# xXCoffeeColaXc/WeatherConverter

Hardware: AMD Instinct MI355X
Metric: 256x256 images/sec (T=1000 DDPM sample) (higher is better)
Workload: dtype fp32-class (f16x3: 2-piece fp16 split MFMA, fp32 accumulate); 1 GPU; DDPM reverse sampling, UNet config.yaml @ 256px, 16 images/GPU, T=1000, 127 timed steps from t=999; global_batch=16, image_size=256, parallelism=single GPU, devices=1, hip_graph=True, stream_groups=2, x_finite=True

## Files before the change

### weatherconverter_amd/csrc/wc_wino.hip

```cpp
#include <stdlib.h>

#include "wc_x6.hpp"

#ifndef WC_ABL
#define WC_ABL 0
#endif
#ifndef WC_WINO_SCALAR
#define WC_WINO_SCALAR 0
#endif

namespace {

using namespace wcx6;

constexpr int NT = 256;

WC_DEVICE void wino_lds16(__amdgpu_buffer_rsrc_t srd, void* dst, unsigned voff, int soff) {
    __builtin_amdgcn_raw_ptr_buffer_load_lds(srd, (__attribute__((address_space(3))) void*)dst, 16, voff, soff, 0, 0);
}

struct WDev {
    const float* src0;
    int C0, ldc0;
    const float* scale;
    const float* shift;
    const float* src1;
    int C1, ldc1;
    int B, H, W, N;
    const void* w;
    const float* bias;
    const float* temb;
    int temb_ld;
    const float* res;
    int ldres;
    float* out;
    int ldo;
    int nck0, nck1;
    int a_exp;
    const float* abound;
    const float* wsinv;
    float* absmax;
    float* gn_part;
    int gn_ncb, gn_sw, gn_c0, gn_np64;
    int tiles_x, tiles_y, ntiles_n;
    const unsigned char* vpre;
    long vimg;
    const float* gb_x;
    int gb_ldx, gb_silu;
    const float* gb_sc0;
    const float* gb_sh0;
    const float* gb_gamma;
    const float* gb_beta;
    float* gb_part;
    float* gb_part3;
};

WC_DEVICE float wino_silu_grad(float y) {
    const float s = 1.0f / (1.0f + __expf(-y));
    return s * (1.0f + y * (1.0f - s));
}

constexpr int VPL = WC_SINGLE16 ? 8 : 16;

template <int TH, int BN, int MB = 2, int NW = 4, bool VP = false>
struct WTile {
    static constexpr int NT = 64 * NW;
    static constexpr int WAVES_N = BN / 32;
    static constexpr int WAVES_M = NW / WAVES_N;
    static_assert(WAVES_N * WAVES_M == NW && WAVES_M * 4 * MB == TH, "each wave owns 4 MB rows x 8 tiles x 32 channels");
    static constexpr int PBN = BN > 128 ? 128 : BN;
    static constexpr int HR = TH + 2;
    static constexpr int PSTR = HR * 128 + (VP ? 0 : 16);
    static constexpr int DPIECES = VPL * HR * 8 / 64;
    static_assert(!VP || VPL * HR * 8 == DPIECES * 64, "VP: the halo stage is a whole number of 1-KiB pieces");
    static constexpr int DPW = (DPIECES + NW - 1) / NW;
    static constexpr int HSTAGE = 16 * PSTR;
    static constexpr int CPSTR = TH * 128 + 16;
    static constexpr int CSTAGE = 8 * CPSTR;
    static constexpr int ITEMS = HR * 16;
    static constexpr int I_PER_T = (ITEMS + NT - 1) / NT;
    static constexpr int C_PER_T = TH * 16 * 4 / NT;
    static constexpr int BSTEP = PBN * 64;
    static constexpr int STEPS = 12;
};

WC_DEVICE int wg_grp(int r) { return ((r >= 4 && r < 12) || (r >= 16 && r < 20) || r >= 28) ? 1 : 0; }
WC_DEVICE int wg_idx(int r) { return r < 4 ? r : r < 12 ? r - 4 : r < 20 ? r - 8 : r < 28 ? r - 12 : r - 16; }
WC_DEVICE int wg_row(int r) { return 2 * wg_grp(r) + (wg_idx(r) >> 3); }
WC_DEVICE int wg_tile(int r) { return wg_idx(r) & 7; }

template <int TH, int BN, int PRO, bool RES, int MB = 2, int NW = 4>
__global__ __launch_bounds__(64 * NW) __attribute__((amdgpu_waves_per_eu(MB == 4 ? 1 : 2, MB == 4 ? 1 : 2)))
void conv3x3_wino_kernel(WDev p) {
    static_assert((PRO == 2 || PRO == 0 || PRO == 3) && !(PRO == 0 && RES),
                  "GN+SiLU (+ residual), pre-split GN+SiLU (+ residual) or one raw segment");
    constexpr bool VP = PRO == 3;
    using T = WTile<TH, BN, MB, NW, VP>;
    constexpr int NT = T::NT;
    extern __shared__ __attribute__((aligned(16))) unsigned char smem[];
    unsigned char* const cbase = smem + 2 * T::HSTAGE;

    const int tid = threadIdx.x;
    const int lane = tid & 63;
    const int wave = tid >> 6;
    const int wm = wave / T::WAVES_N;
    const int wn = wave % T::WAVES_N;

    const int nblk = gridDim.x;
    int bid = blockIdx.x;
    {
        int q = nblk / 8, r = nblk % 8, xcd = bid % 8;
        bid = (xcd < r ? xcd * (q + 1) : r * (q + 1) + (xcd - r) * q) + bid / 8;
    }
    const int tile_n = bid % p.ntiles_n;
    int tt = bid / p.ntiles_n;
    const int txi = tt % p.tiles_x;
    tt /= p.tiles_x;
    const int tyi = tt % p.tiles_y;
    const int b = tt / p.tiles_y;
    const int y0 = tyi * TH, x0 = txi * 16, n0 = tile_n * BN;

    int s_exp = p.a_exp;
    if ((RES || PRO == 0) && p.abound) {
        const float bnd = p.abound[b];
        const int e = (int)((__float_as_uint(bnd) >> 23) & 0xffu) - 127;
        if (bnd > 0.f) s_exp = min(s_exp, (PRO == 0 ? 12 : 13) - e);
        s_exp = max(s_exp, -100);
    }
    const float ascale = ldexpf(1.0f, s_exp), ainv = ldexpf(1.0f, -s_exp);
    const int S0 = T::STEPS * p.nck0;
    const int S = S0 + (RES ? p.nck1 : 0);
    constexpr bool RI = RES && (T::C_PER_T <= 2 || MB == 4);
    const int nri = RI ? min(p.nck0, p.nck1) : 0;
    const int ntail = RES ? p.nck1 - nri : 0;
    constexpr int WPT = T::PBN / 32;
    const unsigned wtile = (unsigned)(tile_n * (BN / T::PBN) + wn / WPT) * (unsigned)(S * T::BSTEP);

    const __amdgpu_buffer_rsrc_t srd0 = make_srd(p.src0);
    const __amdgpu_buffer_rsrc_t srd1 = make_srd(RES ? p.src1 : p.src0);
    const __amdgpu_buffer_rsrc_t srdw = make_srd(p.w);
    const __amdgpu_buffer_rsrc_t srdsc = make_srd(PRO == 2 ? p.scale : p.src0);
    const __amdgpu_buffer_rsrc_t srdsh = make_srd(PRO == 2 ? p.shift : p.src0);
    const __amdgpu_buffer_rsrc_t srdv = make_srd(VP ? (const void*)(p.vpre + (long)b * p.vimg) : (const void*)p.src0);
    unsigned voff[VP ? T::DPW : 1];
    if constexpr (VP) {
#pragma unroll
        for (int i = 0; i < T::DPW; ++i) {
            const int f = (wave + NW * i) * 64 + lane;
            const int P = f / (T::HR * 8), r = (f >> 3) % T::HR, tl = f & 7;
            const int y = y0 - 1 + r;
            voff[i] = (unsigned)y < (unsigned)p.H ? (unsigned)(((P * p.H + y) * (p.W / 2) + (x0 >> 1) + tl) * 16) : OOB;
        }
    }
    const int vchunk = VPL * p.H * (p.W / 2) * 16;
    auto dma_halo = [&](int c, int hs) {
        if constexpr (VP) {
            unsigned char* dst = smem + hs * T::HSTAGE + wave * 1024;
#pragma unroll
            for (int i = 0; i < T::DPW; ++i)
                if (T::DPIECES % NW == 0 || wave + NW * i < T::DPIECES)
                    wino_lds16(srdv, dst + i * NW * 1024, voff[i], c * vchunk);
        }
    };

    const int q = tid & 3;
    int hbase[T::I_PER_T];
    unsigned hin[T::I_PER_T];
    int hwr[T::I_PER_T];
    const int hpx = p.ldc0 * 4;
#pragma unroll
    for (int j = 0; j < T::I_PER_T; ++j) {
        const int i = tid + NT * j;
        const int hrow = i >> 4, tp = (i >> 2) & 3;
        const bool valid = i < T::ITEMS;
        const int iy = y0 - 1 + hrow;
        hin[j] = 0;
#pragma unroll
        for (int k = 0; k < 6; ++k) {
            const int ix = x0 - 1 + 4 * tp + k;
            const bool inb = valid && (unsigned)iy < (unsigned)p.H && (unsigned)ix < (unsigned)p.W;
            hin[j] |= (inb ? 1u : 0u) << k;
        }
        hbase[j] = (((b * p.H + iy) * p.W + x0 - 1 + 4 * tp) * p.ldc0 + 4 * q) * 4;
        hwr[j] = valid ? (q >> 1) * T::PSTR + (hrow * 8 + 2 * tp) * 16 + (q & 1) * 8 : -1;
    }
    f32x4 rh[T::I_PER_T][6];
    f32x4 rsc, rsh;
    auto load_ss = [&](int c) {
        if constexpr (PRO == 2) {
            const unsigned o = (unsigned)(b * p.C0 + c * 16 + 4 * q) * 4u;
            rsc = bload_f4(srdsc, o);
            rsh = bload_f4(srdsh, o);
        }
    };
    auto load_slot = [&](int j, int c) {
#pragma unroll
        for (int k = 0; k < 6; ++k)
            rh[j][k] = bload_f4s(srd0, ((hin[j] >> k) & 1u) ? (unsigned)(hbase[j] + k * hpx) : OOB, c * 64);
    };
    auto load_halo = [&](int c) {
        if constexpr (VP) return;
#pragma unroll
        for (int j = 0; j < T::I_PER_T; ++j) load_slot(j, c);
        load_ss(c);
    };
#if WC_WINO_SCALAR
    const float cu = -1.4426950408889634f * ainv;
    auto prologue = [&](int j, int k0, int k1) {
        if constexpr (PRO == 2) {
            if (j == 0 && k0 == 0) {
                rsc = rsc * ascale;
                rsh = rsh * ascale;
            }
        }
        auto act = [&](f32x4 a) {
#pragma unroll
            for (int e = 0; e < 4; ++e) {
                float v;
                if constexpr (PRO == 2) {
                    const float ap = __builtin_fmaf(a[e], rsc[e], rsh[e]);
                    const float r = __builtin_amdgcn_rcpf(1.0f + __builtin_amdgcn_exp2f(ap * cu));
                    v = ap * r;
                } else {
                    v = a[e] * ascale;
                }
                a[e] = v;
            }
            return a;
        };
#pragma unroll
        for (int k = k0; k < k1; ++k) {
            const f32x4 zero = {0.f, 0.f, 0.f, 0.f};
#if WC_WINO_SCALAR == 2
            rh[j][k] = ((hin[j] >> k) & 1u) ? act(rh[j][k]) : zero;
#else
            const f32x4 a = act(rh[j][k]);
            rh[j][k] = ((hin[j] >> k) & 1u) ? a : zero;
#endif
        }
    };
#else
    auto prologue = [&](int j, int k0, int k1) {
#pragma unroll
        for (int k = k0; k < k1; ++k) {
            f32x4 a = rh[j][k];
            if constexpr (PRO == 2 && !(WC_ABL & 2)) {
                a = a * rsc + rsh;
                if constexpr (!(WC_ABL & 1)) {
                    a.x = silu_fast(a.x); a.y = silu_fast(a.y);
                    a.z = silu_fast(a.z); a.w = silu_fast(a.w);
                }
            }
            rh[j][k] = ((hin[j] >> k) & 1u) ? a * ascale : f32x4{0.f, 0.f, 0.f, 0.f};
        }
    };
#endif
    auto transform = [&](int j, int t, int hs, int p0 = 0, int p1 = 4) {
        if (hwr[j] < 0) return;
        unsigned char* base = smem + hs * T::HSTAGE + hwr[j] + t * 16;
        const f32x4 d0 = rh[j][2 * t], d1 = rh[j][2 * t + 1], d2 = rh[j][2 * t + 2], d3 = rh[j][2 * t + 3];
#if WC_WINO_SCALAR
        f32x4 V[4];
#pragma unroll
        for (int e = 0; e < 4; ++e) {
            V[0][e] = d0[e] - d2[e];
            V[1][e] = d1[e] + d2[e];
            V[2][e] = d2[e] - d1[e];
            V[3][e] = d1[e] - d3[e];
        }
#else
        const f32x4 V[4] = {d0 - d2, d1 + d2, d2 - d1, d1 - d3};
#endif
#pragma unroll
        for (int pos = p0; pos < p1; ++pos) {
            u32x2 a0, a1;
            split2_f16(V[pos], a0, a1);
            unsigned char* d = base + pos * 2 * T::PSTR;
            *reinterpret_cast<u32x2*>(d) = a0;
            *reinterpret_cast<u32x2*>(d + 8 * T::PSTR) = a1;
        }
    };
    auto write_items = [&](int hs) {
        if constexpr (VP) return;
#pragma unroll
        for (int j = 0; j < T::I_PER_T; ++j) {
            prologue(j, 0, 6);
            transform(j, 0, hs);
            transform(j, 1, hs);
        }
    };

    f32x4 rc[2][RES ? T::C_PER_T : 1];
    const int cpx = (tid >> 2) & 15, crow0 = tid >> 6;
    const unsigned coff0 = (unsigned)(((b * p.H + y0 + crow0) * p.W + x0 + cpx) * p.ldc1 + 4 * q);
    const unsigned cstep = (unsigned)(NW * p.W * p.ldc1);
    const int cwr0 = (cpx & 1) * 2 * T::CPSTR + (q >> 1) * T::CPSTR + (crow0 * 8 + (cpx >> 1)) * 16 + (q & 1) * 8;
    auto load_centre = [&](auto P, int c, bool live = true) {
        constexpr int PV = decltype(P)::value;
        const unsigned v = live ? coff0 * 4u : OOB;
#pragma unroll
        for (int j = 0; j < T::C_PER_T; ++j)
            rc[PV][j] = bload_f4s(srd1, v, (int)(((unsigned)j * cstep + (unsigned)c * 16u) * 4u));
    };
    auto write_centre = [&](auto P, int cs) {
        constexpr int PV = decltype(P)::value;
        unsigned char* base = cbase + cs * T::CSTAGE + cwr0;
        const float sg = (cpx & 1) ? -ascale : ascale;
#pragma unroll
        for (int j = 0; j < T::C_PER_T; ++j) {
            u32x2 a0, a1;
            split2_f16(rc[PV][j] * sg, a0, a1);
            unsigned char* d = base + j * NW * 8 * 16;
            *reinterpret_cast<u32x2*>(d) = a0;
            *reinterpret_cast<u32x2*>(d + 4 * T::CPSTR) = a1;
        }
    };

    const int l32 = lane & 31;
    const int half = lane >> 5;
    int abase[MB];
#pragma unroll
    for (int mb = 0; mb < MB; ++mb) abase[mb] = ((4 * MB * wm + 4 * mb + wg_row(l32)) * 8 + wg_tile(l32)) * 16;
    const unsigned wlane = (unsigned)(half * T::PBN * 16 + ((wn % WPT) * 32 + l32) * 16);

    u32x4 wreg[3][2];
    auto load_w = [&](int set, int st) {
        int s = st < S0 ? st : S0 + nri + (st - S0);
        s = s < S ? s : S - 1;
        const int off = (int)(wtile + (unsigned)s * T::BSTEP);
#pragma unroll
        for (int pc = 0; pc < 2; ++pc) wreg[set][pc] = bload_u4s(srdw, wlane + (unsigned)(pc * 2 * T::PBN * 16), off);
    };
    u32x4 wres[2];
    auto load_wres = [&](int r) {
        const int s = S0 + r < S ? S0 + r : S - 1;
        const int off = (int)(wtile + (unsigned)s * T::BSTEP);
#pragma unroll
        for (int pc = 0; pc < 2; ++pc) wres[pc] = bload_u4s(srdw, wlane + (unsigned)(pc * 2 * T::PBN * 16), off);
    };

    f32x16 acc[4][MB];
#pragma unroll
    for (int i = 0; i < 4; ++i)
#pragma unroll
        for (int j = 0; j < MB; ++j)
#pragma unroll
            for (int r = 0; r < 16; ++r) acc[i][j][r] = 0.f;

    u32x4 fa[2][MB][2];
    auto read_a = [&](int fs, int hs, int dy, int pos) {
        const unsigned char* ha = smem + hs * T::HSTAGE + (pos * 2 + half) * T::PSTR + dy * 128;
#pragma unroll
        for (int mb = 0; mb < MB; ++mb)
#pragma unroll
            for (int pc = 0; pc < 2; ++pc)
                fa[fs][mb][pc] = *reinterpret_cast<const u32x4*>(ha + pc * 8 * T::PSTR + abase[mb]);
    };
    auto mfma_a = [&](int fs, int set, int pos) {
#pragma unroll
        for (int mb = 0; mb < MB; ++mb) acc[pos][mb] = mfma_f16(fa[fs][mb][0], wreg[set][0], acc[pos][mb]);
#pragma unroll
        for (int mb = 0; mb < MB; ++mb) {
            acc[pos][mb] = mfma_f16c(fa[fs][mb][0], wreg[set][1], acc[pos][mb]);
            acc[pos][mb] = mfma_f16c(fa[fs][mb][1], wreg[set][0], acc[pos][mb]);
        }
    };
    auto compute_res = [&](const u32x4 (&w)[2], int cs) {
        const unsigned char* ca = cbase + cs * T::CSTAGE + half * T::CPSTR;
#pragma unroll
        for (int r = 0; r < 2; ++r) {
            u32x4 fr[MB][2];
#pragma unroll
            for (int mb = 0; mb < MB; ++mb)
#pragma unroll
                for (int pc = 0; pc < 2; ++pc)
                    fr[mb][pc] = *reinterpret_cast<const u32x4*>(ca + (pc * 4 + r * 2) * T::CPSTR + abase[mb]);
#pragma unroll
            for (int mb = 0; mb < MB; ++mb) {
                f32x16& a = acc[r ? 3 : 0][mb];
                a = mfma_f16(fr[mb][0], w[0], a);
                a = mfma_f16c(fr[mb][0], w[1], a);
                a = mfma_f16c(fr[mb][1], w[0], a);
            }
        }
    };

    const std::integral_constant<int, 0> I0;
    const std::integral_constant<int, 1> I1;
    const int pv0 = (p.nck0 - 1) & 1;
    load_halo(0);
    dma_halo(0, pv0);
    if constexpr (RI) load_centre(I0, 0, nri > 0);
    load_w(0, 0);
    load_w(1, 1);
    write_items(pv0);
    if constexpr (RI) write_centre(I0, pv0);
    if constexpr (VP) asm volatile("s_waitcnt vmcnt(0)" ::: "memory");
    __syncthreads();
    constexpr int HALO_AT = T::I_PER_T == 1 ? 2 : 3;
    auto load_at = [](int j) { return T::I_PER_T == 1 ? 2 : (j == 0 ? 3 : 7); };
    auto pro_at = [](int j) { return j == 0 ? 5 : 9; };
    auto slot_work = [&](int j, int k, int hs) {
        if constexpr (VP) return;
        if constexpr (WC_ABL & 4) {
            if (k >= 0 && k < 3) prologue(j, 2 * k, 2 * k + 2);
            return;
        }
        if constexpr (T::I_PER_T == 1) {
            if (k >= 0 && k < 3) prologue(j, 2 * k, 2 * k + 2);
            if (k >= 3 && k < 7) transform(j, (k - 3) >> 1, hs, ((k - 3) & 1) * 2, ((k - 3) & 1) * 2 + 2);
        } else {
            if (k == 0) prologue(j, 0, 6);
            if (k == 1 || k == 2) transform(j, k - 1, hs);
        }
    };
    auto chunk = [&](auto P, auto L, int c) {
        constexpr int PV = decltype(P)::value;
        constexpr bool LAST = decltype(L)::value != 0;
        read_a(0, PV, 0, 0);
#pragma unroll
        for (int st = 0; st < T::STEPS; ++st) {
            if (!(WC_ABL & 8) || c == 0) load_w((st + 2) % 3, T::STEPS * c + st + 2);
            if constexpr (!LAST) {
#pragma unroll
                for (int j = 0; j < T::I_PER_T; ++j)
                    if (!(WC_ABL & 32) && st == load_at(j)) load_slot(j, c + 1);
                if (st == HALO_AT) {
                    dma_halo(c + 1, PV ^ 1);
                    load_ss(c + 1);
                    if constexpr (RI) load_centre(I0, c + 1, c + 1 < nri);
                }
            } else if constexpr (RES) {
                if (st == HALO_AT) load_centre(I0, nri, ntail > 0);
                if (st == HALO_AT + 1) load_centre(I1, nri + 1, ntail > 1);
            }
            if constexpr (RI) {
                if (st == 9) load_wres(c);
            }
            __builtin_amdgcn_sched_barrier(0);
            if (st + 1 < T::STEPS && (!(WC_ABL & 64) || c == 0)) read_a((st + 1) & 1, PV, (st + 1) >> 2, (st + 1) & 3);
            mfma_a(st & 1, st % 3, st & 3);
            if constexpr (!LAST) {
#pragma unroll
                for (int j = 0; j < T::I_PER_T; ++j) slot_work(j, st - pro_at(j), PV ^ 1);
                if constexpr (RI) {
                    if (st == 9) write_centre(I0, PV ^ 1);
                }
            }
        }
        if constexpr (RES) {
            if constexpr (RI) {
                if (c < nri) compute_res(wres, PV);
            }
            if constexpr (LAST) {
                if (ntail > 0) write_centre(I0, 1);
            }
        }
        if constexpr (VP && !LAST) asm volatile("s_waitcnt vmcnt(4)" ::: "memory");
        if constexpr (!(WC_ABL & 16)) __syncthreads();
    };
    const std::integral_constant<int, 0> NL;
    const std::integral_constant<int, 1> LL;
    {
        int c = 0;
        if (pv0) chunk(I1, NL, c++);
        for (; c + 1 < p.nck0 - 1; c += 2) {
            chunk(I0, NL, c);
            chunk(I1, NL, c + 1);
        }
        chunk(I0, LL, p.nck0 - 1);
    }
    if constexpr (RES) {
        auto tstep = [&](auto P, int k) {
            constexpr int PV = decltype(P)::value;
            compute_res(wreg[PV], PV ^ 1);
            load_w(PV, S0 + k + 2);
            load_centre(P, nri + k + 2, k + 2 < ntail);
            __builtin_amdgcn_sched_barrier(0);
            if (k + 1 < ntail) write_centre(std::integral_constant<int, PV ^ 1>{}, PV);
            __syncthreads();
        };
        int k = 0;
        for (; k + 1 < ntail; k += 2) {
            tstep(I0, k);
            tstep(I1, k + 1);
        }
        if (k < ntail) tstep(I0, k);
    }

    const long img_px = (long)b * p.H * p.W;
    const __amdgpu_buffer_rsrc_t srd_out = make_srd(p.out + img_px * p.ldo);
    const __amdgpu_buffer_rsrc_t srd_res = make_srd(p.res ? p.res + img_px * p.ldres : p.out);
    const int n = n0 + wn * 32 + l32;
    const bool nok = n < p.N;
    float eadd = (nok && p.bias) ? p.bias[n] : 0.f;
    if (nok && p.temb) eadd += p.temb[b * p.temb_ld + n];
    const float emul = nok ? p.wsinv[n] * ainv : 0.f;
    float vmax = 0.f;
    float gs1 = 0.f, gs2 = 0.f, gs3 = 0.f;
    const int so_px = 4 * p.ldo;
    const int so_rs = 4 * p.ldres;
#pragma unroll
    for (int mb = 0; mb < MB; ++mb) {
        unsigned vo[4], vr[4];
#pragma unroll
        for (int j = 0; j < 4; ++j) {
            const int row = 8 * j + 4 * half;
            const int pix = (y0 + 4 * MB * wm + 4 * mb + wg_row(row)) * p.W + x0 + 2 * wg_tile(row);
            vo[j] = (unsigned)(pix * p.ldo + n) * 4u;
            vr[j] = (unsigned)(pix * p.ldres + (nok ? n : 0)) * 4u;
        }
        float rv[2][16];
        if (p.res) {
#pragma unroll
            for (int r = 0; r < 16; ++r) {
                rv[0][r] = bload_f1s(srd_res, vr[r >> 2], (r & 3) * 2 * so_rs);
                rv[1][r] = bload_f1s(srd_res, vr[r >> 2], ((r & 3) * 2 + 1) * so_rs);
            }
        }
#pragma unroll
        for (int r = 0; r < 16; ++r) {
            const float m0 = acc[0][mb][r], m1 = acc[1][mb][r], m2 = acc[2][mb][r], m3 = acc[3][mb][r];
            float ya = ((m0 + m1) + m2) * emul + eadd;
            float yb = ((m1 - m2) - m3) * emul + eadd;
            if (p.res) {
                ya += rv[0][r];
                yb += rv[1][r];
            }
            acc[0][mb][r] = ya;
            acc[1][mb][r] = yb;
            vmax = fmaxf(vmax, fmaxf(fabsf(ya), fabsf(yb)));
        }
        if constexpr (PRO == 0) {
            if (p.gb_part) {
                const __amdgpu_buffer_rsrc_t srd_x = make_srd(p.gb_x + img_px * p.gb_ldx);
                const int so_x = 4 * p.gb_ldx;
                float xv[2][16];
#pragma unroll
                for (int r = 0; r < 16; ++r) {
                    const int j = r >> 2;
                    const int row = 8 * j + 4 * half;
                    const int pix = (y0 + 4 * MB * wm + 4 * mb + wg_row(row)) * p.W + x0 + 2 * wg_tile(row);
                    const unsigned vx = nok ? (unsigned)(pix * p.gb_ldx + n) * 4u : OOB;
                    xv[0][r] = bload_f1s(srd_x, vx, (r & 3) * 2 * so_x);
                    xv[1][r] = bload_f1s(srd_x, vx, ((r & 3) * 2 + 1) * so_x);
                }
                const long bn = (long)b * p.N + (nok ? n : 0);
                const float sc0 = p.gb_sc0[bn], sh0 = p.gb_sh0[bn];
                const float ga = p.gb_gamma ? p.gb_gamma[nok ? n : 0] : 1.f;
                const float be = p.gb_beta ? p.gb_beta[nok ? n : 0] : 0.f;
#pragma unroll
                for (int r = 0; r < 16; ++r)
#pragma unroll
                    for (int e = 0; e < 2; ++e) {
                        const float xh = xv[e][r] * sc0 + sh0;
                        float d = acc[e][mb][r];
                        if (p.gb_silu) d *= wino_silu_grad(ga * xh + be);
                        gs1 += d;
                        gs2 += d * xh;
                        gs3 += xh;
                    }
            }
        }
        if (nok) {
            if constexpr (WC_ABL & 128) {
                float sum = 0.f;
#pragma unroll
                for (int r = 0; r < 16; ++r) sum += acc[0][mb][r] + acc[1][mb][r];
                if (sum == 1234.5678f) bstore_f1s(srd_out, vo[0], 0, sum);
            } else {
#pragma unroll
                for (int r = 0; r < 16; ++r) {
                    bstore_f1s(srd_out, vo[r >> 2], (r & 3) * 2 * so_px, acc[0][mb][r]);
                    bstore_f1s(srd_out, vo[r >> 2], ((r & 3) * 2 + 1) * so_px, acc[1][mb][r]);
                }
            }
        }
    }
    if (!nok) vmax = 0.f;
    if (p.absmax) block_absmax_atomic(p.absmax, b, vmax);
    if constexpr (PRO == 0) {
        if (p.gb_part) {
            gs1 += __shfl_xor(gs1, 32, 64);
            gs2 += __shfl_xor(gs2, 32, 64);
            gs3 += __shfl_xor(gs3, 32, 64);
            const int splits = p.tiles_y * p.tiles_x * T::WAVES_M;
            const long sp = (long)b * splits + ((long)tyi * p.tiles_x + txi) * T::WAVES_M + wm;
            if (nok && half == 0) {
                p.gb_part[(sp * p.N + n) * 2] = gs1;
                p.gb_part[(sp * p.N + n) * 2 + 1] = gs2;
                if (p.gb_part3) p.gb_part3[sp * p.N + n] = gs3;
            }
        }
    }
    if (p.gn_part) {
        const int r4 = tyi * (TH / 4) + MB * wm;
#pragma unroll
        for (int mb = 0; mb < MB; ++mb) {
            const f32x16 blk[2][1] = {{acc[0][mb]}, {acc[1][mb]}};
            GnTile g{p.gn_part, p.gn_ncb, p.gn_sw,
                     (long)b * p.gn_np64 + (long)(((r4 + mb) >> 1) * p.tiles_x + txi) * 2 + ((r4 + mb) & 1),
                     (p.gn_c0 + n0 + wn * 32) / 32};
            gn_tile_partials(blk, g, p.N - n0 - wn * 32 >= 32 ? 1 : 0);
        }
    }
}

template <int TH, int BN, int PRO, bool RES, int MB = 2, int NW = 4>
int launch_wino(const WDev& d, hipStream_t stream) {
    using T = WTile<TH, BN, MB, NW, PRO == 3>;
    constexpr int lds = 2 * T::HSTAGE + (RES ? 2 * T::CSTAGE : 0);
    static bool attr_set = false;
    if (!attr_set) {
        hipError_t e = hipFuncSetAttribute(reinterpret_cast<const void*>(&conv3x3_wino_kernel<TH, BN, PRO, RES, MB, NW>),
                                           hipFuncAttributeMaxDynamicSharedMemorySize, lds);
        if (e != hipSuccess) return (int)e;
        attr_set = true;
    }
    WDev p = d;
    p.tiles_x = p.W / 16;
    p.tiles_y = p.H / TH;
    p.ntiles_n = (p.N + BN - 1) / BN;
    dim3 grid(p.B * p.tiles_y * p.tiles_x * p.ntiles_n);
    WC_SET_NAME("conv3x3_wino_kernel", {WC_TI(TH), WC_TI(BN), WC_TI(PRO), WC_TB(RES), WC_TI(MB), WC_TI(NW)});
    hipLaunchKernelGGL((conv3x3_wino_kernel<TH, BN, PRO, RES, MB, NW>), grid, dim3(T::NT), lds, stream, p);
    WC_CHECK_LAUNCH();
    return WC_OK;
}

}

extern "C" int wc_conv3x3_wino_tile_n(int N) { return N <= 64 ? 64 : 128; }

namespace {

int wino_setup(const wc_conv_args* a, const void* w, int64_t w_bytes, int a_exp, const float* w_inv_scale,
               const float* a_bound, WDev& d, int& pro, bool& res, int& BN) {
    if (!a || !w || !a->out || !w_inv_scale) return WC_E_ARG;
    if (a->nseg < 1 || a->nseg > 2) return WC_E_ARG;
    const wc_conv_seg& s0 = a->seg[0];
    if (!s0.src || (s0.scale == nullptr) != (s0.shift == nullptr)) return WC_E_ARG;
    pro = s0.scale ? 2 : 0;
    if (pro == 2 && !s0.silu) return WC_E_ARG;
    if (pro == 0 && (!a_bound || a->nseg != 1)) return WC_E_ARG;
    if (a->act != WC_ACT_NONE) return WC_E_ARG;
    if (a_exp < -60 || a_exp > 60) return WC_E_ARG;
    BN = wc_conv3x3_wino_tile_n(a->N);
    const int TH = BN == 64 ? 16 : 8;
    if (s0.ntaps != 9 || s0.sy != 1 || s0.sx != 1 || s0.kbase != 0) return WC_E_SHAPE;
    for (int t = 0; t < 9; ++t)
        if (s0.dy[t] != t / 3 - 1 || s0.dx[t] != t % 3 - 1) return WC_E_SHAPE;
    if (s0.C <= 0 || s0.C % 16 || s0.ldc % 4 || (reinterpret_cast<uintptr_t>(s0.src) & 15)) return WC_E_SHAPE;
    if (a->B <= 0 || a->N <= 0 || s0.H != a->Hm || s0.W != a->Wm || a->Hm % TH || a->Wm % 16) return WC_E_SHAPE;
    if ((long)a->B * s0.H * s0.W * s0.ldc * 4 >= (1L << 31)) return WC_E_SHAPE;
    if (reinterpret_cast<uintptr_t>(w) & 15) return WC_E_SHAPE;
    d = WDev{};
    d.src0 = s0.src; d.C0 = s0.C; d.ldc0 = s0.ldc; d.scale = s0.scale; d.shift = s0.shift;
    d.nck0 = s0.C / 16;
    res = a->nseg == 2;
    if (res) {
        const wc_conv_seg& s1 = a->seg[1];
        if (!s1.src || s1.scale || !a_bound) return WC_E_ARG;
        if (s1.ntaps != 1 || s1.dy[0] != 0 || s1.dx[0] != 0 || s1.sy != 1 || s1.sx != 1) return WC_E_SHAPE;
        if (s1.H != s0.H || s1.W != s0.W || s1.kbase != 9 * s0.C) return WC_E_SHAPE;
        if (s1.C <= 0 || s1.C % 16 || s1.ldc % 4 || (reinterpret_cast<uintptr_t>(s1.src) & 15)) return WC_E_SHAPE;
        if ((long)a->B * s1.H * s1.W * s1.ldc * 4 >= (1L << 31)) return WC_E_SHAPE;
        d.src1 = s1.src; d.C1 = s1.C; d.ldc1 = s1.ldc; d.nck1 = s1.C / 16;
    }
    if (a->out_nchw || a->Ho != a->Hm || a->Wo != a->Wm || a->osy != 1 || a->osx != 1 || a->ooy || a->oox)
        return WC_E_SHAPE;
    if ((long)a->Hm * a->Wm * a->ldo * 4 >= (1L << 31) || (a->res && (long)a->Hm * a->Wm * a->ldres * 4 >= (1L << 31)))
        return WC_E_SHAPE;
    d.B = a->B; d.H = a->Hm; d.W = a->Wm; d.N = a->N;
    d.w = w; d.bias = a->bias; d.temb = a->temb; d.temb_ld = a->temb_ld;
    d.res = a->res; d.ldres = a->ldres; d.out = a->out; d.ldo = a->ldo;
    d.a_exp = a_exp - 1;
    d.abound = (res || pro == 0) ? a_bound : nullptr;
    d.wsinv = w_inv_scale;
    d.absmax = a->absmax_out;
    d.gn_part = a->gn_part;
    if (a->gn_part) {
        const int sw = a->gn_sw;
        if ((sw != 4 && sw != 8 && sw != 16 && sw != 32) || a->N % 32 || a->gn_c0 % 32 || a->gn_c0 < 0 ||
            a->gn_c0 + a->N > a->gn_ncb * 32 || a->gn_p64 != 0 || a->gn_np64 * 64 != a->Hm * a->Wm)
            return WC_E_SHAPE;
        d.gn_ncb = a->gn_ncb; d.gn_sw = sw; d.gn_c0 = a->gn_c0; d.gn_np64 = a->gn_np64;
    }
    const long ntn = (a->N + BN - 1) / BN;
    if (w_bytes != ntn * (12L * d.nck0 + d.nck1) * BN * 64 || w_bytes >= (1L << 31)) return WC_E_SHAPE;
    return WC_OK;
}

long wino_vimg(int C, int H, int W) { return (long)(C / 16) * VPL * H * (W / 2) * 16; }

#ifndef VS_IPT
#define VS_IPT 4
#endif
template <int NCK>
__global__ __launch_bounds__(256) void wino_vsplit_kernel(const float* __restrict__ src, int ldc, int B, int H,
                                                          int W, int C, const float* __restrict__ scale,
                                                          const float* __restrict__ shift, int a_exp1,
                                                          const float* __restrict__ res_bound,
                                                          unsigned char* __restrict__ vout, long vimg) {
    extern __shared__ __attribute__((aligned(16))) f32x4 act[];
    const int R = 256 / W, ngrp = C / (16 * NCK), nyb = (H + R - 1) / R;
    const int kg = blockIdx.x % ngrp;
    const int yb = (blockIdx.x / ngrp) % nyb;
    const int b = blockIdx.x / (ngrp * nyb);
    const int y0 = yb * R;
    const int tid = threadIdx.x;
    int s_exp = a_exp1;
    if (res_bound) {
        const float bnd = res_bound[b];
        const int e = (int)((__float_as_uint(bnd) >> 23) & 0xffu) - 127;
        if (bnd > 0.f) s_exp = min(s_exp, 13 - e);
        s_exp = max(s_exp, -100);
    }
    const float ascale = ldexpf(1.0f, s_exp);
    const int W2 = W + 2, items = R * W2 * 4 * NCK, cstride = R * W2 * 5;
    const int qt = tid % (4 * NCK), ct = kg * 16 * NCK + 4 * qt;
    const f32x4 sct = *reinterpret_cast<const f32x4*>(scale + (long)b * C + ct);
    const f32x4 sht = *reinterpret_cast<const f32x4*>(shift + (long)b * C + ct);
    for (int i0 = tid; i0 < items; i0 += VS_IPT * 256) {
        f32x4 v[VS_IPT];
        bool inb[VS_IPT];
        int slot[VS_IPT];
#pragma unroll
        for (int u = 0; u < VS_IPT; ++u) {
            const int i = min(i0 + u * 256, items - 1);
            const int px = (i / (4 * NCK)) % W2 - 1, r = (i / (4 * NCK)) / W2;
            const int y = y0 + r;
            inb[u] = (unsigned)px < (unsigned)W && y < H;
            v[u] = *reinterpret_cast<const f32x4*>(src + ((long)(b * H + min(y, H - 1)) * W + min(max(px, 0), W - 1)) * ldc + ct);
            slot[u] = (qt >> 2) * cstride + (r * W2 + px + 1) * 5 + (qt & 3);
        }
#pragma unroll
        for (int u = 0; u < VS_IPT; ++u) {
            if (i0 + u * 256 >= items) break;
            f32x4 a = v[u] * sct + sht;
            a.x = silu_fast(a.x); a.y = silu_fast(a.y);
            a.z = silu_fast(a.z); a.w = silu_fast(a.w);
            act[slot[u]] = inb[u] ? a * ascale : f32x4{0.f, 0.f, 0.f, 0.f};
        }
    }
    __syncthreads();
    const int T2 = W / 2;
    const int t = tid % T2, h = (tid / T2) & 1, r = tid / W;
    const int y = y0 + r;
    if (r >= R || y >= H) return;
    const long plane = (long)H * T2 * 16;
    const long frag = ((long)y * T2 + t) * 16;
#pragma unroll
    for (int ck = 0; ck < NCK; ++ck) {
        unsigned char* vb = vout + (long)b * vimg + (long)(kg * NCK + ck) * VPL * H * T2 * 16;
        u32x2 pc[2][4][2];
#pragma unroll
        for (int qq = 0; qq < 2; ++qq) {
            const f32x4* ar = act + ck * cstride + (r * W2 + 2 * t) * 5 + 2 * h + qq;
            const f32x4 d0 = ar[0], d1 = ar[5], d2 = ar[10], d3 = ar[15];
            const f32x4 V[4] = {d0 - d2, d1 + d2, d2 - d1, d1 - d3};
#pragma unroll
            for (int pos = 0; pos < 4; ++pos) split2_f16(V[pos], pc[qq][pos][0], pc[qq][pos][1]);
        }
#pragma unroll
        for (int pos = 0; pos < 4; ++pos)
#pragma unroll
            for (int piece = 0; piece < VPL / 8; ++piece)
                *reinterpret_cast<u32x4*>(vb + (piece * 8 + pos * 2 + h) * plane + frag) =
                    u32x4{pc[0][pos][piece].x, pc[0][pos][piece].y, pc[1][pos][piece].x, pc[1][pos][piece].y};
    }
}

}

extern "C" int wc_conv3x3_wino_f16x3(const wc_conv_args* a, const void* w, int64_t w_bytes, int a_exp,
                                     const float* w_inv_scale, const float* a_bound, void* stream) {
    WDev d;
    int pro, BN;
    bool res;
    const int st = wino_setup(a, w, w_bytes, a_exp, w_inv_scale, a_bound, d, pro, res, BN);
    if (st != WC_OK) return st;
    hipStream_t s = reinterpret_cast<hipStream_t>(stream);
    if (pro == 0) return BN == 64 ? launch_wino<16, 64, 0, false>(d, s) : launch_wino<8, 128, 0, false>(d, s);
    if (BN == 64) return res ? launch_wino<16, 64, 2, true>(d, s) : launch_wino<16, 64, 2, false>(d, s);
    return res ? launch_wino<8, 128, 2, true>(d, s) : launch_wino<8, 128, 2, false>(d, s);
}

extern "C" int wc_conv3x3_wino_gnb_splits(int N, int H, int W) {
    const int BN = wc_conv3x3_wino_tile_n(N), TH = BN == 64 ? 16 : 8;
    if (N <= 0 || H <= 0 || W <= 0 || H % TH || W % 16) return -1;
    const int waves_m = 4 / (BN / 32);
    return (H / TH) * (W / 16) * waves_m;
}

extern "C" int wc_conv3x3_wino_f16x3_gnb(const wc_conv_args* a, const void* w, int64_t w_bytes, int a_exp,
                                         const float* w_inv_scale, const float* a_bound, const wc_gnb_epi* g,
                                         void* stream) {
    WDev d;
    int pro, BN;
    bool res;
    const int st = wino_setup(a, w, w_bytes, a_exp, w_inv_scale, a_bound, d, pro, res, BN);
    if (st != WC_OK) return st;
    if (pro != 0 || !g || !g->x || !g->sc0 || !g->sh0 || !g->part) return WC_E_ARG;
    if (g->ldx < d.N || g->splits != wc_conv3x3_wino_gnb_splits(d.N, d.H, d.W)) return WC_E_SHAPE;
    if ((long)d.B * d.H * d.W * g->ldx * 4 >= (1L << 31)) return WC_E_SHAPE;
    d.gb_x = g->x; d.gb_ldx = g->ldx; d.gb_silu = g->silu ? 1 : 0;
    d.gb_sc0 = g->sc0; d.gb_sh0 = g->sh0; d.gb_gamma = g->gamma; d.gb_beta = g->beta;
    d.gb_part = g->part; d.gb_part3 = g->part3;
    hipStream_t s = reinterpret_cast<hipStream_t>(stream);
    return BN == 64 ? launch_wino<16, 64, 0, false>(d, s) : launch_wino<8, 128, 0, false>(d, s);
}

extern "C" int wc_wino_vsplit_bytes(int B, int C, int H, int W, int64_t* bytes) {
    if (!bytes || B <= 0 || C <= 0 || C % 16 || H <= 0 || W <= 0 || W % 16) return WC_E_SHAPE;
    *bytes = (int64_t)B * wino_vimg(C, H, W);
    return WC_OK;
}

extern "C" int wc_wino_vsplit_f16x3(const wc_conv_args* a, int a_exp, const float* a_bound, void* vout, int64_t v_bytes,
                                    void* stream) {
    if (!a || !vout || a->nseg < 1 || a->nseg > 2) return WC_E_ARG;
    const wc_conv_seg& s0 = a->seg[0];
    if (!s0.src || !s0.scale || !s0.shift || !s0.silu) return WC_E_ARG;
    if (a->nseg == 2 && !a_bound) return WC_E_ARG;
    if (a_exp < -60 || a_exp > 60) return WC_E_ARG;
    if (s0.C <= 0 || s0.C % 16 || s0.ldc % 4 || (reinterpret_cast<uintptr_t>(s0.src) & 15) || s0.W % 16)
        return WC_E_SHAPE;
    if ((reinterpret_cast<uintptr_t>(vout) & 15) || v_bytes != (int64_t)a->B * wino_vimg(s0.C, s0.H, s0.W))
        return WC_E_SHAPE;
    if (s0.W > 256) return WC_E_SHAPE;
    const int R = 256 / s0.W;
    const int nck = s0.C % 32 == 0 ? 2 : 1;
    const long nblk = (long)a->B * ((s0.H + R - 1) / R) * (s0.C / (16 * nck));
    const size_t lds = (size_t)nck * R * (s0.W + 2) * 5 * sizeof(f32x4);
    if (lds > 64 * 1024) return WC_E_SHAPE;
    hipStream_t st = reinterpret_cast<hipStream_t>(stream);
    const float* rb = a->nseg == 2 ? a_bound : nullptr;
    unsigned char* vo = reinterpret_cast<unsigned char*>(vout);
    const long vimg = wino_vimg(s0.C, s0.H, s0.W);
    if (nck == 2) {
        WC_SET_NAME("wino_vsplit_kernel", {WC_TI(2)});
        hipLaunchKernelGGL(wino_vsplit_kernel<2>, dim3((unsigned)nblk), dim3(256), lds, st, s0.src, s0.ldc, a->B, s0.H,
                           s0.W, s0.C, s0.scale, s0.shift, a_exp - 1, rb, vo, vimg);
    } else {
        WC_SET_NAME("wino_vsplit_kernel", {WC_TI(1)});
        hipLaunchKernelGGL(wino_vsplit_kernel<1>, dim3((unsigned)nblk), dim3(256), lds, st, s0.src, s0.ldc, a->B, s0.H,
                           s0.W, s0.C, s0.scale, s0.shift, a_exp - 1, rb, vo, vimg);
    }
    WC_CHECK_LAUNCH();
    return WC_OK;
}

extern "C" int wc_conv3x3_wino_f16x3_vp(const wc_conv_args* a, const void* w, int64_t w_bytes, int a_exp,
                                        const float* w_inv_scale, const float* a_bound, const void* vpre,
                                        int64_t v_bytes, void* stream) {
    WDev d;
    int pro, BN;
    bool res;
    const int st = wino_setup(a, w, w_bytes, a_exp, w_inv_scale, a_bound, d, pro, res, BN);
    if (st != WC_OK) return st;
    if (pro != 2 || !vpre || (reinterpret_cast<uintptr_t>(vpre) & 15)) return WC_E_ARG;
    d.vimg = wino_vimg(d.C0, d.H, d.W);
    if (v_bytes != (int64_t)d.B * d.vimg || d.vimg >= (1L << 31)) return WC_E_SHAPE;
    d.vpre = reinterpret_cast<const unsigned char*>(vpre);
    hipStream_t s = reinterpret_cast<hipStream_t>(stream);
    if (BN == 64) return res ? launch_wino<16, 64, 3, true>(d, s) : launch_wino<16, 64, 3, false>(d, s);
    return res ? launch_wino<8, 128, 3, true>(d, s) : launch_wino<8, 128, 3, false>(d, s);
}

extern "C" int wc_conv3x3_wino_f16x3_vp8(const wc_conv_args* a, const void* w, int64_t w_bytes, int a_exp,
                                         const float* w_inv_scale, const float* a_bound, const void* vpre,
                                         int64_t v_bytes, void* stream) {
    WDev d;
    int pro, BN;
    bool res;
    const int st = wino_setup(a, w, w_bytes, a_exp, w_inv_scale, a_bound, d, pro, res, BN);
    if (st != WC_OK) return st;
    if (pro != 2 || !vpre || (reinterpret_cast<uintptr_t>(vpre) & 15)) return WC_E_ARG;
    if (BN != 128 || d.N % 256) return WC_E_SHAPE;
    d.vimg = wino_vimg(d.C0, d.H, d.W);
    if (v_bytes != (int64_t)d.B * d.vimg || d.vimg >= (1L << 31)) return WC_E_SHAPE;
    d.vpre = reinterpret_cast<const unsigned char*>(vpre);
    hipStream_t s = reinterpret_cast<hipStream_t>(stream);
    return res ? launch_wino<8, 256, 3, true, 2, 8>(d, s) : launch_wino<8, 256, 3, false, 2, 8>(d, s);
}

namespace {

__device__ double wino_u(const float* row, int C0, int ky, int pos, int c) {
    const double g0 = row[(ky * 3 + 0) * C0 + c], g1 = row[(ky * 3 + 1) * C0 + c], g2 = row[(ky * 3 + 2) * C0 + c];
    switch (pos) {
        case 0: return g0;
        case 1: return ((g0 + g1) + g2) * 0.5;
        case 2: return ((g0 - g1) + g2) * 0.5;
        default: return g2;
    }
}

__device__ void wino_u8(const float* row, int ld, int ky, int pos, int c, double* v) {
    f32x4 g[3][2];
#pragma unroll
    for (int k = 0; k < 3; ++k) {
        g[k][0] = *reinterpret_cast<const f32x4*>(row + (ky * 3 + k) * ld + c);
        g[k][1] = *reinterpret_cast<const f32x4*>(row + (ky * 3 + k) * ld + c + 4);
    }
#pragma unroll
    for (int e = 0; e < 8; ++e) {
        const double g0 = g[0][e >> 2][e & 3], g1 = g[1][e >> 2][e & 3], g2 = g[2][e >> 2][e & 3];
        v[e] = pos == 0 ? g0 : pos == 1 ? ((g0 + g1) + g2) * 0.5 : pos == 2 ? ((g0 - g1) + g2) * 0.5 : g2;
    }
}

__device__ void pack_wino_row(const float* row3, int ld, bool vec, const float* rres, bool live, int n, int C0, int C1,
                              int BN, short* __restrict__ out, float* __restrict__ wsinv) {
    const int c8 = C0 / 8, n0 = 12 * c8, nall = n0 + C1 / 8;
    auto values = [&](int it, double* v) {
        if (it < n0) {
            const int kp = it / c8, c = (it - kp * c8) * 8;
            if (vec) {
                wino_u8(row3, ld, kp / 4, kp % 4, c, v);
            } else {
#pragma unroll
                for (int e = 0; e < 8; ++e) v[e] = wino_u(row3, ld, kp / 4, kp % 4, c + e);
            }
        } else {
            const int c = (it - n0) * 8;
#pragma unroll
            for (int e = 0; e < 8; ++e) v[e] = rres[c + e];
        }
    };
    double m = 0.0;
    if (live) {
        for (int it = threadIdx.x; it < nall; it += blockDim.x) {
            double v[8];
            values(it, v);
#pragma unroll
            for (int e = 0; e < 8; ++e) m = fmax(m, fabs(v[e]));
        }
    }
    __shared__ double red[256];
    red[threadIdx.x] = m;
    __syncthreads();
    for (int s = 128; s > 0; s >>= 1) {
        if ((int)threadIdx.x < s) red[threadIdx.x] = fmax(red[threadIdx.x], red[threadIdx.x + s]);
        __syncthreads();
    }
    const double amax = red[0];
    int sw = 0;
    if (amax > 0.0) {
        int e;
        const double mant = frexp(amax, &e);
        sw = (mant == 0.5 ? 15 : 14) - e;
        sw = sw < -60 ? -60 : sw > 60 ? 60 : sw;
    }
    const double scale = ldexp(1.0, sw);
    if (threadIdx.x == 0) wsinv[n] = ldexpf(1.0f, -sw);
    const int T = n / BN, nn = n % BN;
    const long rowlen = (long)(12 * (C0 / 16) + C1 / 16) * 2 * 2 * BN * 8;
    short* trow = out + (long)T * rowlen;
    const int plane = 2 * BN * 8;
    for (int it = threadIdx.x; it < nall; it += blockDim.x) {
        double v[8];
        if (live) values(it, v);
        else
#pragma unroll
            for (int e = 0; e < 8; ++e) v[e] = 0.0;
        long o;
        if (it < n0) {
            const int kp = it / c8, c = (it - kp * c8) * 8, ky = kp / 4, pos = kp % 4;
            const int chunk = c / 16, kh = (c % 16) / 8;
            o = ((((long)(chunk * 3 + ky) * 4 + pos) * 2 * 2 + kh) * BN + nn) * 8;
        } else {
            const int c = (it - n0) * 8;
            const int chunk = c / 16, kh = (c % 16) / 8;
            o = (long)(C0 / 16) * 12 * 2 * 2 * BN * 8 + (((long)chunk * 2 * 2 + kh) * BN + nn) * 8;
        }
        unsigned hp[4], lp[4];
#pragma unroll
        for (int e = 0; e < 8; e += 2) {
            unsigned short h0, l0, h1, l1;
            float a = (float)(v[e] * scale), b = (float)(v[e + 1] * scale);
            asm volatile("" : "+v"(a), "+v"(b));
            split2_one(a, h0, l0);
            split2_one(b, h1, l1);
            hp[e / 2] = (unsigned)h0 | ((unsigned)h1 << 16);
            lp[e / 2] = (unsigned)l0 | ((unsigned)l1 << 16);
        }
        *reinterpret_cast<u32x4*>(trow + o) = u32x4{hp[0], hp[1], hp[2], hp[3]};
        *reinterpret_cast<u32x4*>(trow + o + plane) = u32x4{lp[0], lp[1], lp[2], lp[3]};
    }
}

__global__ __launch_bounds__(256) void pack_wino_kernel(const float* __restrict__ w, int K, int N, int C0, int C1,
                                                        int BN, short* __restrict__ out, float* __restrict__ wsinv) {
    const int n = blockIdx.x;
    const bool live = n < N;
    const float* row = w + (long)(live ? n : 0) * K;
    pack_wino_row(row, C0, false, row + 9 * C0, live, n, C0, C1, BN, out, wsinv);
}

__device__ void stage_row3(const float* __restrict__ w, bool transposed, int N, int n, int C0, float* row3) {
    const int lim = 9 * C0, ld = C0 + 4;
    for (int i0 = threadIdx.x; i0 < lim; i0 += 8 * 256) {
        float v[8];
#pragma unroll
        for (int k = 0; k < 8; ++k) {
            const int i = i0 + k * 256;
            const int c = i / 9, t = i - 9 * c;
            v[k] = i < lim ? (transposed ? w[((long)c * N + n) * 9 + t] : w[(long)n * lim + i]) : 0.f;
        }
#pragma unroll
        for (int k = 0; k < 8; ++k) {
            const int i = i0 + k * 256;
            const int c = i / 9, t = i - 9 * c;
            if (i < lim) row3[(transposed ? 8 - t : t) * ld + c] = v[k];
        }
    }
}

template <bool TRANSPOSED>
__global__ __launch_bounds__(256) void pack_wino_raw_kernel(const float* __restrict__ w, const float* __restrict__ wres,
                                                            int N, int C0, int C1, int BN, short* __restrict__ out,
                                                            float* __restrict__ wsinv) {
    extern __shared__ float row3[];
    const int n = blockIdx.x;
    const bool live = n < N;
    if (live) stage_row3(w, TRANSPOSED, N, n, C0, row3);
    __syncthreads();
    pack_wino_row(row3, C0 + 4, true, wres + (long)(live ? n : 0) * C1, live, n, C0, C1, BN, out, wsinv);
}

__global__ __launch_bounds__(256) void pack_wino_batch_kernel(const wc_wino_pack_job* __restrict__ jobs, int njobs) {
    extern __shared__ float row3[];
    __shared__ int s_wg0[256];
    const int g = blockIdx.x;
    const bool lds = njobs <= 256;
    if (lds && (int)threadIdx.x < njobs) s_wg0[threadIdx.x] = jobs[threadIdx.x].wg0;
    __syncthreads();
    int lo = 0, hi = njobs - 1;
    while (lo < hi) {
        const int mid = (lo + hi + 1) >> 1;
        if ((lds ? s_wg0[mid] : jobs[mid].wg0) <= g) lo = mid;
        else hi = mid - 1;
    }
    const wc_wino_pack_job jb = jobs[lo];
    const int n = g - jb.wg0;
    const bool live = n < jb.N;
    const int C0 = jb.C0, N = jb.N;
    if (live) stage_row3(jb.w, jb.transposed != 0, N, n, C0, row3);
    __syncthreads();
    pack_wino_row(row3, C0 + 4, true, jb.wres + (long)(live ? n : 0) * jb.C1, live, n, C0, jb.C1, jb.BN,
                  reinterpret_cast<short*>(jb.out), jb.wsinv);
}

}

extern "C" int wc_pack_wino(const float* w, int N, int C0, int C1, void* out, int64_t out_bytes, float* w_inv_scale,
                            void* stream) {
    if (!w || !out || !w_inv_scale) return WC_E_ARG;
    if (N <= 0 || C0 <= 0 || C0 % 16 || C1 < 0 || C1 % 16) return WC_E_SHAPE;
    const int BN = wc_conv3x3_wino_tile_n(N);
    const long ntn = (N + BN - 1) / BN;
    if (out_bytes != ntn * (12L * (C0 / 16) + C1 / 16) * BN * 64) return WC_E_SHAPE;
    hipLaunchKernelGGL(pack_wino_kernel, dim3((unsigned)(ntn * BN)), dim3(256), 0, reinterpret_cast<hipStream_t>(stream),
                       w, 9 * C0 + C1, N, C0, C1, BN, reinterpret_cast<short*>(out), w_inv_scale);
    wc_last_kernel = "pack_wino_kernel";
    WC_CHECK_LAUNCH();
    return WC_OK;
}

extern "C" int wc_pack_wino_batch(const wc_wino_pack_job* jobs, int njobs, int total_wg, int max_c0, void* stream) {
    if (!jobs || njobs < 0 || total_wg < 0) return WC_E_ARG;
    if (njobs == 0) return WC_OK;
    if (max_c0 <= 0 || 9L * (max_c0 + 4) * 4 > 64 * 1024 || total_wg <= 0) return WC_E_SHAPE;
    hipLaunchKernelGGL(pack_wino_batch_kernel, dim3((unsigned)total_wg), dim3(256), (size_t)9 * (max_c0 + 4) * sizeof(float),
                       reinterpret_cast<hipStream_t>(stream), jobs, njobs);
    wc_last_kernel = "pack_wino_batch_kernel";
    WC_CHECK_LAUNCH();
    return WC_OK;
}

extern "C" int wc_pack_wino_raw(const float* w, const float* wres, int N, int C0, int C1, int transposed, void* out,
                                int64_t out_bytes, float* w_inv_scale, void* stream) {
    if (!w || !out || !w_inv_scale || (C1 && !wres) || (transposed && C1)) return WC_E_ARG;
    if (N <= 0 || C0 <= 0 || C0 % 16 || C1 < 0 || C1 % 16 || 9L * (C0 + 4) * 4 > 64 * 1024) return WC_E_SHAPE;
    const int BN = wc_conv3x3_wino_tile_n(N);
    const long ntn = (N + BN - 1) / BN;
    if (out_bytes != ntn * (12L * (C0 / 16) + C1 / 16) * BN * 64) return WC_E_SHAPE;
    const size_t lds = (size_t)9 * (C0 + 4) * sizeof(float);
    hipStream_t s = reinterpret_cast<hipStream_t>(stream);
    if (transposed)
        hipLaunchKernelGGL(pack_wino_raw_kernel<true>, dim3((unsigned)(ntn * BN)), dim3(256), lds, s, w, wres, N, C0, C1,
                           BN, reinterpret_cast<short*>(out), w_inv_scale);
    else
        hipLaunchKernelGGL(pack_wino_raw_kernel<false>, dim3((unsigned)(ntn * BN)), dim3(256), lds, s, w, wres, N, C0,
                           C1, BN, reinterpret_cast<short*>(out), w_inv_scale);
    wc_last_kernel = "pack_wino_raw_kernel";
    WC_CHECK_LAUNCH();
    return WC_OK;
}
```

Before: 0.6939 images/s.

## Add optional staggered two-half K-loop schedule with triple-buffered halo for VP8 Winograd

Adds a compile-time-gated schedule for the 8-wave pre-split Winograd conv. In it, half the waves lag the other half by part of a chunk, so MFMA and DMA/LDS phases overlap across wave groups, using a 3-slot halo/centre ring. A constexpr checker validates barrier counts and slot reuse. The wave index is also forced uniform via readfirstlane, which is on by default, while the stagger itself is off by default. The stagger costs extra LDS and a more complex barrier protocol.

```diff
diff --git a/weatherconverter_amd/csrc/wc_wino.hip b/weatherconverter_amd/csrc/wc_wino.hip
--- a/weatherconverter_amd/csrc/wc_wino.hip
+++ b/weatherconverter_amd/csrc/wc_wino.hip
@@ -7,6 +7,15 @@
 #endif
 #ifndef WC_WINO_SCALAR
 #define WC_WINO_SCALAR 0
+#endif
+#ifndef WC_WINO_VP8_STAGGER
+#define WC_WINO_VP8_STAGGER 0
+#endif
+#ifndef WC_WINO_VP8_LAG
+#define WC_WINO_VP8_LAG 6
+#endif
+#ifndef WC_WINO_VP8_UWAVE
+#define WC_WINO_VP8_UWAVE 1
 #endif
 
 namespace {
@@ -82,12 +91,73 @@
     static constexpr int C_PER_T = TH * 16 * 4 / NT;
     static constexpr int BSTEP = PBN * 64;
     static constexpr int STEPS = 12;
+    static constexpr bool STAG = VP && NW == 8 && WC_WINO_VP8_STAGGER;
+    static constexpr int RING = STAG ? 3 : 2;
 };
+
+template <int LAG_>
+struct WStag {
+    static constexpr int LAG = LAG_, STEPS = 12, RING = 3;
+    static constexpr int DMA_PH = 2, CW_PH = 9, WRES_ST = 9;
+    static constexpr int phase(int half, int st) { return half ? (st + STEPS - LAG) % STEPS : st; }
+    static_assert(LAG >= 1 && LAG < STEPS, "half 1 lags by part of a chunk");
+    static_assert(STEPS - LAG <= CW_PH && DMA_PH + 1 <= STEPS - 1 - LAG, "LAG 3 .. 8 with these phases");
+    static_assert(phase(1, WRES_ST) < STEPS - 2 && DMA_PH + 1 < STEPS - 2, "only weight loads in the last two phases");
+    static constexpr int slot(int c) { return c % RING; }
+    static constexpr int begin(int half, int k) { return half && k ? STEPS * (k - 1) + LAG : STEPS * k; }
+    static constexpr int end(int half, int k, int n) { return half && k < n - 1 ? STEPS * k + LAG : STEPS * (k + 1); }
+    static constexpr int barriers(int half, int n, int ntail) {
+        int nb = 1;
+        if (half == 0) {
+            for (int c = 0; c + 1 < n; ++c) ++nb;
+        } else {
+            for (int k = 1; k < n; ++k) ++nb;
+        }
+        if (ntail > 0) nb += 1 + ntail;
+        return nb;
+    }
+    static constexpr bool reads(int half, int k, int n, int s) {
+        if (k >= n) return slot(k) == s;
+        for (int g = begin(half, k); g < end(half, k, n); ++g)
+            if (slot(g / STEPS) == s) return true;
+        return false;
+    }
+    static constexpr bool ok(int n, int ntail) {
+        if (barriers(0, n, ntail) != barriers(1, n, ntail)) return false;
+        for (int half = 0; half < 2; ++half) {
+            int g = 0;
+            for (int k = 0; k < n; ++k) {
+                if (begin(half, k) != g || end(half, k, n) <= g) return false;
+                g = end(half, k, n);
+            }
+            if (g != STEPS * n) return false;
+        }
+        for (int k = 0; k < n + ntail - 1; ++k)
+            for (int half = 0; half < 2; ++half)
+                if (reads(half, k, n, slot(k + 1))) return false;
+        for (int half = 0; half < 2; ++half)
+            for (int k = 0; k < n; ++k)
+                for (int g = begin(half, k); g < end(half, k, n); ++g)
+                    if (g / STEPS > k) return false;
+        for (int half = 0; half < 2; ++half)
+            if (reads(half, n - 1, n, slot(n))) return false;
+        return true;
+    }
+    static constexpr bool ok_all() {
+        for (int n = 1; n <= 8; ++n)
+            for (int ntail = 0; ntail <= 5; ++ntail)
+                if (!ok(n, ntail)) return false;
+        return true;
+    }
+};
+static_assert(WStag<WC_WINO_VP8_LAG>::ok_all(), "staggered schedule: barrier counts, step order or slot reuse");
 
 WC_DEVICE int wg_grp(int r) { return ((r >= 4 && r < 12) || (r >= 16 && r < 20) || r >= 28) ? 1 : 0; }
 WC_DEVICE int wg_idx(int r) { return r < 4 ? r : r < 12 ? r - 4 : r < 20 ? r - 8 : r < 28 ? r - 12 : r - 16; }
 WC_DEVICE int wg_row(int r) { return 2 * wg_grp(r) + (wg_idx(r) >> 3); }
 WC_DEVICE int wg_tile(int r) { return wg_idx(r) & 7; }
+
+WC_DEVICE int wino_uniform(int v) { return __builtin_amdgcn_readfirstlane(v); }
 
 template <int TH, int BN, int PRO, bool RES, int MB = 2, int NW = 4>
 __global__ __launch_bounds__(64 * NW) __attribute__((amdgpu_waves_per_eu(MB == 4 ? 1 : 2, MB == 4 ? 1 : 2)))
@@ -98,11 +168,11 @@
     using T = WTile<TH, BN, MB, NW, VP>;
     constexpr int NT = T::NT;
     extern __shared__ __attribute__((aligned(16))) unsigned char smem[];
-    unsigned char* const cbase = smem + 2 * T::HSTAGE;
+    unsigned char* const cbase = smem + T::RING * T::HSTAGE;
 
     const int tid = threadIdx.x;
     const int lane = tid & 63;
-    const int wave = tid >> 6;
+    const int wave = (VP && NW == 8 && WC_WINO_VP8_UWAVE) ? wino_uniform(tid >> 6) : tid >> 6;
     const int wm = wave / T::WAVES_N;
     const int wn = wave % T::WAVES_N;
 
@@ -153,13 +223,13 @@
         }
     }
     const int vchunk = VPL * p.H * (p.W / 2) * 16;
-    auto dma_halo = [&](int c, int hs) {
+    auto dma_halo = [&](int c, int hs, bool live = true) {
         if constexpr (VP) {
             unsigned char* dst = smem + hs * T::HSTAGE + wave * 1024;
 #pragma unroll
             for (int i = 0; i < T::DPW; ++i)
                 if (T::DPIECES % NW == 0 || wave + NW * i < T::DPIECES)
-                    wino_lds16(srdv, dst + i * NW * 1024, voff[i], c * vchunk);
+                    wino_lds16(srdv, dst + i * NW * 1024, live ? voff[i] : OOB, live ? c * vchunk : 0);
         }
     };
 
@@ -388,15 +458,17 @@
     const std::integral_constant<int, 0> I0;
     const std::integral_constant<int, 1> I1;
     const int pv0 = (p.nck0 - 1) & 1;
-    load_halo(0);
-    dma_halo(0, pv0);
-    if constexpr (RI) load_centre(I0, 0, nri > 0);
-    load_w(0, 0);
-    load_w(1, 1);
-    write_items(pv0);
-    if constexpr (RI) write_centre(I0, pv0);
-    if constexpr (VP) asm volatile("s_waitcnt vmcnt(0)" ::: "memory");
-    __syncthreads();
+    if constexpr (!T::STAG) {
+        load_halo(0);
+        dma_halo(0, pv0);
+        if constexpr (RI) load_centre(I0, 0, nri > 0);
+        load_w(0, 0);
+        load_w(1, 1);
+        write_items(pv0);
+        if constexpr (RI) write_centre(I0, pv0);
+        if constexpr (VP) asm volatile("s_waitcnt vmcnt(0)" ::: "memory");
+        __syncthreads();
+    }
     constexpr int HALO_AT = T::I_PER_T == 1 ? 2 : 3;
     auto load_at = [](int j) { return T::I_PER_T == 1 ? 2 : (j == 0 ? 3 : 7); };
     auto pro_at = [](int j) { return j == 0 ? 5 : 9; };
@@ -461,7 +533,7 @@
     };
     const std::integral_constant<int, 0> NL;
     const std::integral_constant<int, 1> LL;
-    {
+    if constexpr (!T::STAG) {
         int c = 0;
         if (pv0) chunk(I1, NL, c++);
         for (; c + 1 < p.nck0 - 1; c += 2) {
@@ -470,7 +542,7 @@
         }
         chunk(I0, LL, p.nck0 - 1);
     }
-    if constexpr (RES) {
+    if constexpr (RES && !T::STAG) {
         auto tstep = [&](auto P, int k) {
             constexpr int PV = decltype(P)::value;
             compute_res(wreg[PV], PV ^ 1);
@@ -488,6 +560,124 @@
         if (k < ntail) tstep(I0, k);
     }
 
+    if constexpr (T::STAG) {
+        using SP = WStag<WC_WINO_VP8_LAG>;
+        constexpr int LAG = SP::LAG;
+        const bool lagging = wino_uniform(wave) >= NW / 2;
+        static_assert(VP && T::I_PER_T == 1 && HALO_AT == SP::DMA_PH && SP::STEPS == T::STEPS && SP::RING == T::RING &&
+                          (RI || !RES), "the plan describes this tile's K loop");
+        const int n = p.nck0;
+        auto nx = [](int s) { return s == SP::RING - 1 ? 0 : s + 1; };
+        auto kwin = [&](auto H_, auto A_, auto B_, auto HK_, auto PRE_, int c, int sl, int k, int slw, int slp) {
+            constexpr int H = decltype(H_)::value;
+            constexpr int A = decltype(A_)::value, B = decltype(B_)::value, HK = decltype(HK_)::value;
+            constexpr bool PRE = decltype(PRE_)::value != 0;
+#pragma unroll
+            for (int st = A; st < B; ++st) {
+                const int ph = SP::phase(H, st);
+                load_w((st + 2) % 3, T::STEPS * c + st + 2);
+                if constexpr (HK == 1) {
+                    if (ph == SP::DMA_PH) {
+                        dma_halo(k + 1, slw, k + 1 < n);
+                        if constexpr (RI) load_centre(I0, k + 1, k + 1 < nri);
+                    }
+                } else if constexpr (RES) {
+                    if (ph == SP::DMA_PH) load_centre(I0, nri, ntail > 0);
+                    if (ph == SP::DMA_PH + 1) load_centre(I1, nri + 1, ntail > 1);
+                }
+                if constexpr (RI) {
+                    if (st == SP::WRES_ST) load_wres(c);
+                }
+                __builtin_amdgcn_sched_barrier(0);
+                if (st + 1 < T::STEPS) read_a((st + 1) & 1, sl, (st + 1) >> 2, (st + 1) & 3);
+                else if constexpr (PRE) read_a(0, slp, 0, 0);
+                mfma_a(st & 1, st % 3, st & 3);
+                if constexpr (HK == 1 && RI) {
+                    if (ph == SP::CW_PH) write_centre(I0, slw);
+                }
+            }
+        };
+        auto rendezvous = [&]() {
+            asm volatile("s_waitcnt vmcnt(4)" ::: "memory");
+            __syncthreads();
+        };
+        const std::integral_constant<int, 0> C0;
+        const std::integral_constant<int, 1> C1;
+        const std::integral_constant<int, 2> C2;
+        const std::integral_constant<int, LAG> CLAG;
+        const std::integral_constant<int, T::STEPS> CEND;
+        dma_halo(0, 0);
+        if constexpr (RI) load_centre(I0, 0, nri > 0);
+        load_w(0, 0);
+        load_w(1, 1);
+        if constexpr (RI) write_centre(I0, 0);
+        asm volatile("s_waitcnt vmcnt(0)" ::: "memory");
+        int tsl;
+        if (!lagging) {
+            __syncthreads();
+            int sl = 0;
+            for (int c = 0; c + 1 < n; ++c) {
+                read_a(0, sl, 0, 0);
+                kwin(C0, C0, CEND, C1, C0, c, sl, c, nx(sl), 0);
+                if constexpr (RI) {
+                    if (c < nri) compute_res(wres, sl);
+                }
+                rendezvous();
+                sl = nx(sl);
+            }
+            read_a(0, sl, 0, 0);
+            kwin(C0, C0, CEND, C2, C0, n - 1, sl, n - 1, 0, 0);
+            if constexpr (RI) {
+                if (n - 1 < nri) compute_res(wres, sl);
+            }
+            tsl = nx(sl);
+        } else {
+            __syncthreads();
+            int sp = 0, sc = 0;
+            read_a(0, 0, 0, 0);
+            dma_halo(1, 1, 1 < n);
+            if constexpr (RI) load_centre(I0, 1, 1 < nri);
+            kwin(C1, C0, CLAG, C1, C0, 0, 0, 0, 1, 0);
+            for (int k = 1; k < n; ++k) {
+                sp = sc;
+                sc = nx(sc);
+                rendezvous();
+                kwin(C1, CLAG, CEND, C1, C1, k - 1, sp, k, nx(sc), sc);
+                if constexpr (RI) {
+                    if (k - 1 < nri) compute_res(wres, sp);
+                }
+                kwin(C1, C0, CLAG, C1, C0, k, sc, k, nx(sc), 0);
+            }
+            kwin(C1, CLAG, CEND, C2, C0, n - 1, sc, n - 1, 0, 0);
+            if constexpr (RI) {
+                if (n - 1 < nri) compute_res(wres, sc);
+            }
+            tsl = nx(sc);
+        }
+        if constexpr (RES) {
+            if (ntail > 0) {
+                write_centre(I0, tsl);
+                __syncthreads();
+                auto tstep = [&](auto P, int k, int sr) {
+                    constexpr int PV = decltype(P)::value;
+                    compute_res(wreg[PV], sr);
+                    load_w(PV, S0 + k + 2);
+                    load_centre(P, nri + k + 2, k + 2 < ntail);
+                    __builtin_amdgcn_sched_barrier(0);
+                    if (k + 1 < ntail) write_centre(std::integral_constant<int, PV ^ 1>{}, nx(sr));
+                    __syncthreads();
+                };
+                int k = 0, sr = tsl;
+                for (; k + 1 < ntail; k += 2) {
+                    tstep(I0, k, sr);
+                    tstep(I1, k + 1, nx(sr));
+                    sr = nx(nx(sr));
+                }
+                if (k < ntail) tstep(I0, k, sr);
+            }
+        }
+    }
+
     const long img_px = (long)b * p.H * p.W;
     const __amdgpu_buffer_rsrc_t srd_out = make_srd(p.out + img_px * p.ldo);
     const __amdgpu_buffer_rsrc_t srd_res = make_srd(p.res ? p.res + img_px * p.ldres : p.out);
@@ -609,7 +799,7 @@
 template <int TH, int BN, int PRO, bool RES, int MB = 2, int NW = 4>
 int launch_wino(const WDev& d, hipStream_t stream) {
     using T = WTile<TH, BN, MB, NW, PRO == 3>;
-    constexpr int lds = 2 * T::HSTAGE + (RES ? 2 * T::CSTAGE : 0);
+    constexpr int lds = T::RING * T::HSTAGE + (RES ? T::RING * T::CSTAGE : 0);
     static bool attr_set = false;
     if (!attr_set) {
         hipError_t e = hipFuncSetAttribute(reinterpret_cast<const void*>(&conv3x3_wino_kernel<TH, BN, PRO, RES, MB, NW>),
```

New measurement: 0.7008 images/s, median of 6. Within noise of the previous version (+1.0%).
